# openfheorg/openfhe-development

Measured on AMD Instinct MI355X. Metric: NTT GB/s vs HBM roofline + CKKS EvalMultKeySwitch/sec, N=2^16 L=30, 1/2/4/8 GPU, higher is better.
Workload: dtype u64; 1 GPU; batched fwd+inv negacyclic NTT, N=2^16, L=30 x 60-bit limbs, 1024 polynomials per GPU (BASELINE configs[1]); global_batch=1024, parallelism=batch-sharded x1, no data-path collective

## Files before the change

### openfhe-development_amd/csrc/fhe_hip.cpp

```cpp
#include "../../include/fhe_hip.h"

#include <algorithm>
#include <cmath>
#include <cstdio>
#include <cstdlib>
#include <map>
#include <mutex>
#include <shared_mutex>
#include <string>
#include <type_traits>
#include <vector>

#include "basis_kernels.h"
#include "bfv_kernels.h"
#include "elemwise_kernels.h"
#include "host_math.h"
#include "ntt_kernels.h"
#include "ntt_static.h"
#include "ntt_row8.h"
#include "rt.h"
#include "sampler_kernels.h"
#include "blake2_kernels.h"

using namespace fhe;
// ... 447 lines not shown
    ARG_CHECK(c && graph, "fhe_graph_launch: null argument");
    RT_CHECK(rt::graph_launch((rt::graph_t)graph, (rt::stream_t)stream));
    return FHE_OK;
}
extern "C" void fhe_graph_destroy(void* graph) {
    if (graph)
        rt::graph_destroy((rt::graph_t)graph);
}

static fhe_status make_sel(const fhe_ctx* c, const uint32_t* limbIdx, uint32_t nLimbs, LimbSel* sel, const char* who) {
    if (nLimbs < 1 || nLimbs > (uint32_t)kMaxLimbs)
        return fail(FHE_ERR_ARG, std::string(who) + ": nLimbs out of range");
    for (uint32_t i = 0; i < nLimbs; ++i) {
        uint32_t l = limbIdx ? limbIdx[i] : i;
        if (l >= c->L)
            return fail(FHE_ERR_ARG, std::string(who) + ": limb index exceeds context size");
        sel->idx[i] = (uint8_t)l;
    }
    for (uint32_t i = nLimbs; i < (uint32_t)kMaxLimbs; ++i)
        sel->idx[i] = 0;
    return FHE_OK;
}
static inline uint32_t tiles_for(const fhe_ctx* c, uint64_t rows) {
    const uint64_t words = rows << c->logN;
    return (uint32_t)((words + kTile - 1) >> kTileLog);
}
#define LAUNCH_CHECK() RT_CHECK(rt::last_launch_error())

static uint32_t env_u32(const char* name, uint32_t dflt) {
    const char* v = std::getenv(name);
    return v ? (uint32_t)std::strtoul(v, nullptr, 10) : dflt;
}
constexpr bool kHandoverDefault = true;
struct NttSwitches {
    int row8 = -1, row8X1 = -1;
    uint32_t row8Batch = 0, t1 = 0;
    bool handover = kHandoverDefault;
};
static const NttSwitches& ntt_switches() {
    static const NttSwitches sw = [] {
        NttSwitches s;
        auto flag = [](const char* name) {
            const char* v = std::getenv(name);
            return v && (v[0] == '0' || v[0] == '1') ? v[0] - '0' : -1;
        };
        s.row8   = flag("FHE_NTT_ROW8");
        s.row8X1 = flag("FHE_NTT_ROW8_X1");
        if (const char* v = std::getenv("FHE_NTT_ROW8_BATCH"))
            s.row8Batch = (v[0] == '1' || v[0] == '2' || v[0] == '4') && !v[1] ? (uint32_t)(v[0] - '0') : 0u;
        if (const char* v = std::getenv("FHE_NTT_HANDOVER")) {
            s.handover = v[0] == '1' && !v[1];
            if (!s.handover && !(v[0] == '0' && !v[1]))
                fprintf(stderr, "fhe_hip: FHE_NTT_HANDOVER=%s is neither 0 nor 1: hand-over is off\n", v);
        }
        s.t1 = env_u32("FHE_NTT_T1", 0);
        return s;
    }();
    return sw;
}
static bool row8_for(uint32_t T) { return ntt_switches().row8 >= 0 ? ntt_switches().row8 == 1 : T <= 11u; }
constexpr uint32_t kRow8BatchDefault = 2;
constexpr bool kRow8X1RegionsP2 = false, kRow8X1RegionsP4 = false;
static uint32_t row8_batch_for(uint32_t T) {
    if (T != 12u)
        return 1u;
    return ntt_switches().row8Batch ? ntt_switches().row8Batch : ntt_switches().row8 >= 0 ? 1u : kRow8BatchDefault;
}
static bool row8_x1_regions(uint32_t P) {
    return ntt_switches().row8X1 >= 0 ? ntt_switches().row8X1 == 1 : (P == 2 ? kRow8X1RegionsP2 : kRow8X1RegionsP4);
}
static uint32_t ntt_t1(uint32_t logN) {
    const uint32_t forced = ntt_switches().t1;
    if (forced >= 4 && forced <= 5 && logN > (uint32_t)kTileLog && logN - forced >= 9 && logN - forced <= 12)
        return forced;
    return std::max(4u, logN - (uint32_t)kTileLog);
}

struct NttPass {
    enum Kind { Single, Column, Row };
    bool inverse = false;
    Kind kind    = Single;
    uint32_t T   = 0;
    int mode = 1;
    NttPass() = default;
    NttPass(bool inv, Kind k, uint32_t stages) : inverse(inv), kind(k), T(stages), mode(k == Row ? (inv ? 0 : 9) : 1) {}
    bool layoutA() const { return kind == Column; }
};
struct NttPasses {
// ... 122 lines not shown
    FHE_INSTANCE(FHE_PASS_IS(LA, INV, TT, MODE), FHE_LAUNCH_BARRIER((ntt_static_kernel<LA, INV, TT, MODE>), pass_tiles(*a), stream, *a))
    FHE_CASE(true, false, 4, 1) FHE_CASE(true, true, 4, 1) FHE_CASE(true, false, 5, 1) FHE_CASE(true, true, 5, 1)
    FHE_CASE(false, false, 12, 9) FHE_CASE(false, true, 12, 0) FHE_CASE(false, false, 11, 9) FHE_CASE(false, true, 11, 0)
    FHE_CASE(false, false, 10, 9) FHE_CASE(false, true, 10, 0) FHE_CASE(false, false, 9, 9) FHE_CASE(false, true, 9, 0)
    FHE_CASE(false, false, 12, 1) FHE_CASE(false, true, 12, 1)
#undef FHE_CASE
    return false;
}
static bool static_epilogue_instance(const NttPass& p, const NttPassArgs* a, void* stream) {
#define FHE_CASE(TT, MODE) \
    FHE_INSTANCE(FHE_PASS_IS(false, false, TT, MODE),                                                                                \
                 FHE_LAUNCH_AS("EPI", (ntt_static_kernel<false, false, TT, MODE, true>), pass_tiles(*a), kThreads, true, stream, *a))
    FHE_CASE(12, 9) FHE_CASE(11, 9) FHE_CASE(10, 9) FHE_CASE(9, 9) FHE_CASE(12, 1)
#undef FHE_CASE
    return false;
}
static bool static_prologue_instance(const NttPass& p, const NttPassArgs* a, void* stream) {
#define FHE_CASE(TT)                                                                                                                  \
    FHE_INSTANCE(FHE_PASS_IS(true, false, TT, 1) && !(a && a->proMode >= 2u),                                                         \
                 FHE_LAUNCH_AS("PRO", (ntt_static_kernel<true, false, TT, 1, false, 1>), pass_tiles(*a), kThreads, true, stream, *a))  \
    FHE_INSTANCE(FHE_PASS_IS(true, false, TT, 1) && a && a->proMode == 2u,                                                            \
                 FHE_LAUNCH_AS("PRO2", (ntt_static_kernel<true, false, TT, 1, false, 2>), pass_tiles(*a), kThreads, true, stream, *a)) \
    FHE_INSTANCE(FHE_PASS_IS(true, false, TT, 1) && a && a->proMode == 3u,                                                            \
                 FHE_LAUNCH_AS("PRO3", (ntt_static_kernel<true, false, TT, 1, false, 3>), pass_tiles(*a), kThreads, true, stream, *a))
    FHE_CASE(4) FHE_CASE(5)
#undef FHE_CASE
    return false;
}
static bool static_handover_instance(const NttPass& p, const NttPassArgs* a, void* stream) {
    FHE_INSTANCE(FHE_PASS_IS(true, true, 4, 1), FHE_LAUNCH_AS("HAND", (ntt_static_kernel<true, true, 4, 1, false, false, true>), pass_tiles(*a),
                                                              kThreads, true, stream, *a))
    return false;
}
static NttPassArgs row8_args(const NttPassArgs& a, uint32_t P) {
    NttPassArgs r = a;
    r.batch       = a.batch / P;
    r.rows        = r.batch * a.nLimbs;
    r.xcdSwizzle  = ((a.nLimbs << (a.logN - a.T)) % 8u == 0) ? 1u : 0u;
    return r;
}
static bool row8_instance(const NttPass& p, const NttPassArgs* a, void* stream) {
#define FHE_CASE(INV, TT, MODE)                                                                                                       \
    FHE_INSTANCE(FHE_PASS_IS(false, INV, TT, MODE), FHE_LAUNCH_BARRIER_N((r8::ntt_row8_kernel<INV, TT - 9, MODE>), a->rows << (a->logN - TT), \
                                                                         64u << (TT - 9), stream, *a))
    FHE_CASE(false, 12, 9) FHE_CASE(true, 12, 0) FHE_CASE(false, 11, 9) FHE_CASE(true, 11, 0)
    FHE_CASE(false, 10, 9) FHE_CASE(true, 10, 0) FHE_CASE(false, 9, 9) FHE_CASE(true, 9, 0)
#undef FHE_CASE
    return false;
}
static bool row8_batched_instance(const NttPass& p, uint32_t P, bool hand, const NttPassArgs* a, void* stream) {
    const bool x1p = row8_x1_regions(P);
#define FHE_CASE(INV, MODE, PP, X1P)                                                                                                  \
    FHE_INSTANCE(FHE_PASS_IS(false, INV, 12, MODE) && P == PP && x1p == X1P && !hand,                                                 \
                 FHE_LAUNCH_BARRIER_N((r8::ntt_row8_batched_kernel<INV, 3, MODE, PP, X1P>), a->rows << (a->logN - 12), 512u, stream, *a))      \
    FHE_INSTANCE(INV && FHE_PASS_IS(false, INV, 12, MODE) && P == PP && x1p == X1P && hand,                                           \
                 FHE_LAUNCH_AS("HAND", (r8::ntt_row8_batched_kernel<INV, 3, MODE, PP, X1P, INV>), a->rows << (a->logN - 12), 512u, true, stream, \
                               *a))
    FHE_CASE(false, 9, 2, false) FHE_CASE(true, 0, 2, false) FHE_CASE(false, 9, 2, true) FHE_CASE(true, 0, 2, true)
    FHE_CASE(false, 9, 4, false) FHE_CASE(true, 0, 4, false) FHE_CASE(false, 9, 4, true) FHE_CASE(true, 0, 4, true)
#undef FHE_CASE
    return false;
}
static bool poly_mul_instance(const NttPass& p, bool second, const PolyMulArgs* a, void* stream) {
#define FHE_CASE(TT)                                                                                                                \
    FHE_INSTANCE(FHE_PASS_IS(false, false, TT, 9) && !second, FHE_LAUNCH_BARRIER((poly_mul_row_a_kernel<TT>), pass_tiles(a->fwd), stream, *a)) \
    FHE_INSTANCE(FHE_PASS_IS(false, false, TT, 9) && second, FHE_LAUNCH_BARRIER((poly_mul_row_b_kernel<TT>), pass_tiles(a->fwd), stream, *a))
    FHE_CASE(12) FHE_CASE(11) FHE_CASE(10) FHE_CASE(9)
#undef FHE_CASE
    return false;
}
#undef FHE_INSTANCE
#undef FHE_PASS_IS

static bool ntt_epilogue_supported(const fhe_ctx* c) {
    const NttPasses f = ntt_passes(c, false);
    return static_epilogue_instance(f.p[f.n - 1], nullptr, nullptr);
}
static bool ntt_prologue_supported(const fhe_ctx* c) {
    const NttPasses f = ntt_passes(c, false);
    return f.n == 2 && static_prologue_instance(f.p[0], nullptr, nullptr);
}

static void fill_pass_args(const fhe_ctx* c, const NttPass& p, const uint64_t* xin, uint64_t* xout, const LimbSel& sel, uint32_t nLimbs,
                           uint32_t batch, const NttOpts& o, NttPassArgs& a) {
    a.outStride = o.dst.stride;
    a.outFirst  = o.dst.first;
    a.inStride  = o.src.stride;
    a.inFirst   = o.src.first;
    a.inDelta   = o.srcDelta;
    a.xin       = xin;
    a.x         = xout;
    a.tw        = p.inverse ? c->d_twInv : c->d_tw;
    a.twRow     = p.inverse ? c->d_twRowInv : c->d_twRow;
    a.q         = c->d_q;
    a.red       = c->d_red;
    a.fin       = c->d_fin;
    a.logN      = c->logN;
    a.T         = p.T;
    a.nLimbs    = nLimbs;
    a.rows      = batch * nLimbs;
    a.batch     = batch;
    a.nSteps = a.canonLevels = 0;
    a.canonStep              = o.canonOut ? 0u : 0xffffffffu;
    for (NttStep& st : a.steps)
        st = NttStep{0, 0, -1, 0, 0, 0, 0, 0};
    a.sel = sel;
    const uint32_t tilesPerRow = c->N >= (uint32_t)kTile ? (c->N >> kTileLog) : 1u;
    a.xcdSwizzle = (c->N >= (uint32_t)kTile && ((nLimbs * tilesPerRow) % 8u == 0)) ? 1u : 0u;
    static const NttEpilogue noEpi;
    const NttEpilogue& e = o.epi && o.epi->mode ? *o.epi : noEpi;
    a.epiMode = e.mode, a.epiSplit = e.split, a.epiAStride = e.aStride, a.epiAFirst = e.aFirst;
    a.epiA = e.A, a.epiC = e.C, a.epiOut0 = e.out0, a.epiOut1 = e.out1, a.epiADelta = e.aDelta;
    a.proMode = o.proSrcLimb ? (o.proRows ? 3 : o.proC ? 2 : 1) : 0, a.proSrcLimb = o.proSrcLimb ? *o.proSrcLimb : 0;
    a.proC = o.proSrcLimb ? o.proC : nullptr;
    a.proRows = o.proSrcLimb ? o.proRows : 0;
    for (uint32_t k = 0; k < 4; ++k)
        a.proSrcLimbs[k] = k < a.proRows ? o.proSrcLimb[k] : 0;
}
static NttPassArgs split_head(NttPassArgs& a, uint32_t n) {
    NttPassArgs h = a;
    h.batch       = n;
    h.rows        = n * a.nLimbs;
    a.xin += a.inDelta ? (int64_t)n * a.inDelta : (int64_t)(((uint64_t)n * (a.inStride ? a.inStride : a.nLimbs)) << a.logN);
    a.x += ((uint64_t)n * (a.outStride ? a.outStride : a.nLimbs)) << a.logN;
    a.batch -= n;
    a.rows = a.batch * a.nLimbs;
    return h;
}
static fhe_status launch_pass(const fhe_ctx* c, const NttPass& p, const uint64_t* xin, uint64_t* xout, const LimbSel& sel, uint32_t nLimbs,
                              uint32_t batch, void* stream, const NttOpts& o = NttOpts(), uint32_t handP = 0) {
    NttPassArgs a;
    fill_pass_args(c, p, xin, xout, sel, nLimbs, batch, o, a);
    enum { Small, Static, Epilogue, Prologue, Row8 } rest = c->logN < (uint32_t)kTileLog ? Small : Static;
    uint32_t headP = 0;
    if (o.srcDelta && rest == Small)
        return fail(FHE_ERR_UNSUPPORTED, "ntt: separately allocated towers need a ring of at least 4096");
    if (o.proSrcLimb) {
        rest = Prologue;
        if (!static_prologue_instance(p, nullptr, nullptr))
            return fail(FHE_ERR_UNSUPPORTED, "ntt: no prologue kernel for this pass shape");
    }
    else if (a.epiMode) {
        rest = Epilogue;
        if (!static_epilogue_instance(p, nullptr, nullptr))
            return fail(FHE_ERR_UNSUPPORTED, "ntt: no epilogue kernel for this pass shape");
    }
    else if (rest != Small) {
        const uint32_t P = p.kind == NttPass::Row ? row8_batch_for(p.T) : 1u;
        if (handP && !(batch >= handP && (p.layoutA() ? static_handover_instance(p, nullptr, nullptr)
                                                      : P == handP && row8_batched_instance(p, P, true, nullptr, nullptr))))
            return fail(FHE_ERR_UNSUPPORTED, "ntt: no hand-over kernel for this pass shape");
        if (handP && p.layoutA())
            headP = handP;
        else if (P > 1 && batch >= P && row8_batched_instance(p, P, handP != 0, nullptr, nullptr))
            headP = P;
        if (p.kind == NttPass::Row && row8_for(p.T) && row8_instance(p, nullptr, nullptr))
            rest = Row8;
        else if (!static_instance(p, nullptr, nullptr))
            return fail(FHE_ERR_UNSUPPORTED, "ntt: no kernel instance for this pass shape");
    }
    if (headP) {
        NttPassArgs h = split_head(a, batch / headP * headP);
        if (p.layoutA())
            static_handover_instance(p, &h, stream);
        else
            h = row8_args(h, headP), row8_batched_instance(p, headP, handP != 0, &h, stream);
    }
    if (a.batch)
        switch (rest) {
            case Static: static_instance(p, &a, stream); break;
            case Epilogue: static_epilogue_instance(p, &a, stream); break;
            case Prologue: static_prologue_instance(p, &a, stream); break;
            case Row8: a = row8_args(a, 1), row8_instance(p, &a, stream); break;
            case Small: launch_small(p, o.canonOut, a, stream); break;
        }
    LAUNCH_CHECK();
    return FHE_OK;
}

static fhe_status ntt_run(fhe_ctx* c, bool inverse, const uint64_t* xin, uint64_t* xout, const uint32_t* limbIdx, uint32_t nLimbs,
                          uint32_t batch, void* stream, const NttOpts& o = NttOpts()) {
    ARG_CHECK(c && xin && xout, "fhe_ntt: null argument");
    ARG_CHECK(batch >= 1, "fhe_ntt: batch must be >= 1");
    LimbSel sel;
    if (fhe_status s = make_sel(c, limbIdx, nLimbs, &sel, "fhe_ntt"))
        return s;
    RT_CHECK(rt::set_device(c->device));
    const NttPasses ps = ntt_passes(c, inverse);
    if (ps.n == 1)
        return launch_pass(c, ps.p[0], xin, xout, sel, nLimbs, batch, stream, o);
    const uint32_t rowP  = inverse ? row8_batch_for(ps.p[0].T) : 1u;
    const uint32_t handP = (o.canonOut && !(o.epi && o.epi->mode) && !o.proSrcLimb && ntt_switches().handover && rowP >= 2 &&
                            batch >= rowP && row8_batched_instance(ps.p[0], rowP, true, nullptr, nullptr) &&
                            static_handover_instance(ps.p[1], nullptr, nullptr))
                               ? rowP
                               : 0u;
    NttOpts first = o, second;
    first.epi = nullptr, first.canonOut = false;
    second.src = second.dst = o.dst;
    second.epi = o.epi, second.canonOut = o.canonOut;
    if (fhe_status s = launch_pass(c, ps.p[0], xin, xout, sel, nLimbs, batch, stream, first, handP))
        return s;
    return launch_pass(c, ps.p[1], xout, xout, sel, nLimbs, batch, stream, second, handP);
}

extern "C" fhe_status fhe_ntt_fwd(fhe_ctx* c, uint64_t* x, const uint32_t* li, uint32_t nl, uint32_t b, void* st) {
    return ntt_run(c, false, x, x, li, nl, b, st);
}
extern "C" fhe_status fhe_ntt_inv(fhe_ctx* c, uint64_t* x, const uint32_t* li, uint32_t nl, uint32_t b, void* st) {
    return ntt_run(c, true, x, x, li, nl, b, st);
}
extern "C" fhe_status fhe_ntt_fwd_oop(fhe_ctx* c, const uint64_t* xi, uint64_t* xo, const uint32_t* li, uint32_t nl,
                                      uint32_t b, void* st) {
    return ntt_run(c, false, xi, xo, li, nl, b, st);
}
extern "C" fhe_status fhe_ntt_inv_oop(fhe_ctx* c, const uint64_t* xi, uint64_t* xo, const uint32_t* li, uint32_t nl,
                                      uint32_t b, void* st) {
    return ntt_run(c, true, xi, xo, li, nl, b, st);
}

extern "C" size_t fhe_poly_mul_workspace_bytes(const fhe_ctx* c, uint32_t nLimbs, uint32_t batch) {
    return c ? (((size_t)2 * batch * nLimbs) << c->logN) * 8 : 0;
}
extern "C" fhe_status fhe_poly_mul(fhe_ctx* c, const uint64_t* a, const uint64_t* b, uint64_t* out, const uint32_t* limbIdx,
                                   uint32_t nLimbs, uint32_t batch, void* wsv, size_t wsBytes, void* stream) {
    ARG_CHECK(c && a && b && out && wsv, "fhe_poly_mul: null argument");
    ARG_CHECK(batch >= 1, "fhe_poly_mul: batch must be >= 1");
    ARG_CHECK(wsBytes >= fhe_poly_mul_workspace_bytes(c, nLimbs, batch), "fhe_poly_mul: workspace too small");
    LimbSel sel;
    if (fhe_status s = make_sel(c, limbIdx, nLimbs, &sel, "fhe_poly_mul"))
        return s;
    RT_CHECK(rt::set_device(c->device));
    uint64_t* wa = (uint64_t*)wsv;
    uint64_t* wb = wa + (((size_t)batch * nLimbs) << c->logN);
    const NttPasses f = ntt_passes(c, false), i = ntt_passes(c, true);
    if (f.n != 2 || !poly_mul_instance(f.p[1], false, nullptr, nullptr)) {
// ... 3936 lines not shown
```

### openfhe-development_amd/csrc/ntt_kernels.h

```cpp
#ifndef FHE_NTT_KERNELS_H
#define FHE_NTT_KERNELS_H
#include "modarith.h"
#include "launch.h"

namespace fhe {

constexpr int kTileLog  = 12;
constexpr int kTile     = 1 << kTileLog;
constexpr int kThreads  = 256;
constexpr int kMaxLimbs = 256;

struct alignas(16) TwPair {
    uint64_t w, wp;
};

struct LimbSel {
    uint8_t idx[kMaxLimbs];
};

struct NttStep {
    int8_t fI;
    int8_t Fj;
    int8_t bHi;
    int8_t bLo;
// ... 4 lines not shown
};

struct NttPassArgs {
    const uint64_t* xin;
    uint64_t* x;
    const TwPair* tw;
    const TwPair* twRow;
    const uint64_t* q;
    const uint64_t* red;
    const TwPair* fin;
    uint32_t logN;
    uint32_t T;
    uint32_t nLimbs;
    uint32_t rows;
    uint32_t batch;
    uint32_t nSteps;
    uint32_t canonLevels;
    uint32_t canonStep;
    uint32_t xcdSwizzle;
    uint32_t inStride;
    uint32_t inFirst;
    uint32_t outStride;
    uint32_t outFirst;
    NttStep steps[6];
    LimbSel sel;
    uint32_t epiMode, epiSplit, epiAStride, epiAFirst;
    const uint64_t* epiA;
    const TwPair* epiC;
    uint64_t *epiOut0, *epiOut1;
    uint32_t proMode, proSrcLimb;
    const TwPair* proC;
    uint32_t proRows, proSrcLimbs[4];
    int64_t inDelta, epiADelta;
};
FHE_HD uint64_t switch_modulus_word(uint64_t v, uint64_t qs, uint64_t halfQs, uint64_t qn) {
    if (qn > qs)
        return v + ((v > halfQs) ? (qn - qs) : 0);
    uint64_t bv = (v > halfQs) ? (qs - qn) : 0;
    uint64_t av = v;
    if (av >= qn)
        av %= qn;
    if (bv >= qn)
        bv %= qn;
    return (av < bv) ? av + qn - bv : av - bv;
}

FHE_HD uint32_t lds_sigma(uint32_t I) {
    return I ^ ((I >> 4) & 31u);
}

FHE_HD void bfly_fwd(uint64_t& a, uint64_t& b, const TwPair w, uint64_t nq, uint64_t twoq) {
    uint64_t X = csub(a, twoq);
    uint64_t T = mul_shoup_lazy_nq(b, w.w, w.wp, nq);
    a          = X + T;
    b          = X - T + twoq;
}
FHE_HD void bfly_inv(uint64_t& a, uint64_t& b, const TwPair w, uint64_t nq, uint64_t twoq) {
    uint64_t u = a, v = b;
    a          = csub(u + v, twoq);
    b          = mul_shoup_lazy_nq(u - v + twoq, w.w, w.wp, nq);
}
FHE_HD void bfly_inv_last(uint64_t& a, uint64_t& b, const TwPair nInv, const TwPair w1nInv, uint64_t nq,
                          uint64_t twoq) {
    uint64_t u = a, v = b;
    a          = mul_shoup_lazy_nq(u + v, nInv.w, nInv.wp, nq);
    b          = mul_shoup_lazy_nq(u - v + twoq, w1nInv.w, w1nInv.wp, nq);
// ... 216 lines not shown
```

### openfhe-development_amd/csrc/ntt_row8.h

```cpp
#ifndef FHE_NTT_ROW8_H
#define FHE_NTT_ROW8_H
#include "ntt_static.h"
#include "ntt_bfly8_pinned.h"
#include <type_traits>
#if defined(__HIP_DEVICE_COMPILE__) && !defined(FHE_NO_BFLY_ASM)
namespace fhe {
namespace r8 {
#define FHE_BK 1
namespace bk1 {
#include "ntt_bfly8_banked.h"
}
#undef FHE_BK
#define FHE_BK 2
namespace bk2 {
#include "ntt_bfly8_banked.h"
}
#undef FHE_BK
#define FHE_BK 3
namespace bk3 {
#include "ntt_bfly8_banked.h"
}
#undef FHE_BK
}
}
// ... 214 lines not shown
}
template <bool UNI, int NB, bool SWEEP>
FHE_HD void fwd_step(uint64_t (&r)[8], const TwPair* tw, uint32_t hi, uint32_t F, uint32_t logN, const BflyConst c, uint32_t inBound) {
    uint32_t bnd[8];
    for (int k = 0; k < 8; ++k)
        bnd[k] = inBound;
    TwPair w2[4], w1[4], w0[4];
    if constexpr (NB >= 1) load_tw<UNI, 2>(w2, tw, hi, F, logN);
    if constexpr (NB >= 2) load_tw<UNI, 1>(w1, tw, hi, F, logN);
    if constexpr (SWEEP && NB >= 1)
        red4_a<2>(r, c, bnd);
    if constexpr (NB >= 1) fwd_stage<UNI, 2>(r, w2, c, bnd);
    if constexpr (NB >= 3) load_tw<UNI, 0>(w0, tw, hi, F, logN);
    if constexpr (NB >= 2) fwd_stage<UNI, 1>(r, w1, c, bnd);
    if constexpr (NB >= 3) fwd_stage<UNI, 0>(r, w0, c, bnd);
}
template <bool UNI, int NB, bool LAZY>
FHE_HD void inv_step(uint64_t (&r)[8], const TwPair* tw, uint32_t hi, uint32_t F, uint32_t logN, const BflyConst c) {
    uint32_t bnd[8];
    for (int k = 0; k < 8; ++k)
        bnd[k] = 3;
    TwPair w2[4], w1[4], w0[4];
    if constexpr (NB >= 3) load_tw<UNI, 0>(w0, tw, hi, F, logN);
    if constexpr (NB >= 2) load_tw<UNI, 1>(w1, tw, hi, F, logN);
    if constexpr (NB >= 1 && NB < 3) load_tw<UNI, 2>(w2, tw, hi, F, logN);
    if constexpr (NB >= 3) inv_stage<UNI, NB, 0>(r, w0, c, bnd);
    if constexpr (NB >= 3) load_tw<UNI, 2>(w2, tw, hi, F, logN);
    if constexpr (NB >= 2) inv_stage<UNI, NB, 1>(r, w1, c, bnd);
    if constexpr (NB >= 1) inv_stage<UNI, NB, 2>(r, w2, c, bnd);
    if constexpr (!LAZY && NB >= 1)
        inv_end<NB>(r, c, bnd);
}

template <int WB, int BIN>
struct FwdSched {
    static constexpr int TA = WB;
    static constexpr int stages(int i) { return i == 0 ? TA : 3; }
    static constexpr int before(int i) {
        int b = BIN;
        for (int j = 0; j < i; ++j)
            b = (b + 3 * stages(j) <= 16) ? b + 3 * stages(j) : 2 + 3 * stages(j);
        return b;
    }
    static constexpr bool sweep(int i) { return before(i) + 3 * stages(i) > 16; }
    static constexpr int out = before(4);
};

struct TileAt {
    uint32_t tb, rit, tr;
};
FHE_DEV TileAt tile_at(const NttPassArgs& a, uint32_t vt, uint32_t trLog, bool swz) {
    uint32_t tile = vt;
    if (swz) {
        const uint32_t xcd = vt & 7u, i = vt >> 3;
        const uint32_t b = i % a.batch, pairIdx = i / a.batch;
        const uint32_t pair = pairIdx * 8u + xcd;
        tile = ((b * a.nLimbs + (pair >> trLog)) << trLog) + (pair & ((1u << trLog) - 1u));
    }
    const uint32_t row = tile >> trLog;
    return TileAt{row / a.nLimbs, row % a.nLimbs, tile & ((1u << trLog) - 1u)};
}

#if defined(__HIP_DEVICE_COMPILE__)
#define FHE_R8_OPAQUE_V(x) asm volatile("" : "+v"(x))
#else
#define FHE_R8_OPAQUE_V(x) ((void)0)
#endif
#define FHE_R8_LANE()                 \
    uint32_t tq_ = t;                 \
// ... 218 lines not shown
    if constexpr (NB >= 3) load_tw<UNI, 0>(w0, tw, hi, F, logN);
    FHE_R8_BANKS(p)
        if constexpr (NB >= 2) fwd_stage<UNI, 1, p>(r[p], w1, c, bnd[p]);
    FHE_R8_BANKS_END
    FHE_R8_BANKS(p)
        if constexpr (NB >= 3) fwd_stage<UNI, 0, p>(r[p], w0, c, bnd[p]);
    FHE_R8_BANKS_END
}
template <bool UNI, int NB, bool LAZY, int P, bool HAND = false>
FHE_HD void inv_step_b(uint64_t (&r)[P][8], const TwPair* tw, uint32_t hi, uint32_t F, uint32_t logN, const BflyConst c) {
    uint32_t bnd[P][8];
    for (int p = 0; p < P; ++p)
        for (int k = 0; k < 8; ++k)
            bnd[p][k] = 3;
    TwPair w2[4], w1[4], w0[4];
    if constexpr (NB >= 3) load_tw<UNI, 0>(w0, tw, hi, F, logN);
    if constexpr (NB >= 2) load_tw<UNI, 1>(w1, tw, hi, F, logN);
    if constexpr (NB >= 1 && NB < 3) load_tw<UNI, 2>(w2, tw, hi, F, logN);
    FHE_R8_BANKS(p)
        if constexpr (NB >= 3) inv_stage<UNI, NB, 0, p>(r[p], w0, c, bnd[p]);
    FHE_R8_BANKS_END
    static_assert(!HAND || (NB == 3 && LAZY), "row8 hand-over: the boundary stage is the last of the full step that closes a lazy-out pass");
    if constexpr (NB >= 3 && !HAND) load_tw<UNI, 2>(w2, tw, hi, F, logN);
    FHE_R8_BANKS(p)
        if constexpr (NB >= 2) inv_stage<UNI, NB, 1, p>(r[p], w1, c, bnd[p]);
    FHE_R8_BANKS_END
    FHE_R8_BANKS(p)
        if constexpr (HAND) inv_stage_hand<p>(r[p], c, bnd[p]);
        else if constexpr (NB >= 1) inv_stage<UNI, NB, 2, p>(r[p], w2, c, bnd[p]);
        if constexpr (!LAZY && NB >= 1) inv_end<NB, p>(r[p], c, bnd[p]);
    FHE_R8_BANKS_END
}

template <bool INV, int WB, int MODE, int P, bool X1P, bool HAND = false>
FHE_DEV void ntt_row8_batched_core(const NttPassArgs& a, uint64_t* lds) {
    static_assert(WB == 3, "row8 batched: 8 waves per tile (12 stages): the banked blocks exist for full radix-8 steps only");
    static_assert(P >= 2 && P <= 4, "row8 batched: register banks 0..3");
    static_assert(!(INV && MODE != 0), "row8: the inverse pass that ends a transform is ntt_static.h's");
    static_assert(!HAND || INV, "row8 hand-over: the inverse pass only");
    constexpr uint32_t tileLog = 9u + (uint32_t)WB;
    constexpr uint32_t threads = 64u << WB;
    constexpr int WLOW         = 3 - WB;
    constexpr uint32_t x1Set   = X1P ? (uint32_t)kRegion << WB : 0u;
    const uint32_t t     = FHE_TID;
    const uint32_t wv    = FHE_UNIFORM(t >> 6);
    const uint32_t logN  = a.logN;
    const uint32_t trLog = logN - tileLog;
    uint64_t* reg = lds + (size_t)wv * kRegion;
    uint64_t r[P][8];
    const TileAt at      = tile_at(a, FHE_BID, trLog, a.xcdSwizzle != 0);
    const uint32_t jbase = at.tr << tileLog;
    const uint32_t rit   = at.rit;
    const uint32_t tb0   = at.tb * (uint32_t)P;
    const uint64_t inRow  = a.inStride ? ((uint64_t)tb0 * a.inStride + a.inFirst + rit) : ((uint64_t)tb0 * a.nLimbs + rit);
    const uint64_t outRow = a.outStride ? ((uint64_t)tb0 * a.outStride + a.outFirst + rit) : ((uint64_t)tb0 * a.nLimbs + rit);
    const uint32_t limb = FHE_UNIFORM(a.sel.idx[rit]);
    const uint64_t q    = FHE_ULOAD64(a.q, limb);
    const uint64_t twoq = q << 1, nq = 0 - q;
    const TwPair* tw    = a.tw + ((uint64_t)limb << logN);
    const uint64_t redc = FHE_ULOAD64(a.red, limb);
    const BflyConst c{(uint32_t)nq, (uint32_t)(nq >> 32), q, twoq, 0 - twoq, twoq + q, (uint32_t)redc, (uint32_t)(redc >> 32)};
    const uint64_t* src = (a.inDelta ? a.xin + (int64_t)tb0 * a.inDelta + ((uint64_t)(a.inFirst + rit) << logN) : a.xin + (inRow << logN)) + jbase;
    uint64_t* dst       = a.x + (outRow << logN) + jbase;
    const int64_t inStep  = a.inDelta ? a.inDelta : (int64_t)((uint64_t)(a.inStride ? a.inStride : a.nLimbs) << logN);
    const int64_t outStep = (int64_t)((uint64_t)(a.outStride ? a.outStride : a.nLimbs) << logN);
    auto x1 = [](int rr) { return (uint32_t)kRegion * ((uint32_t)rr >> WLOW) + (64u << WB) * ((uint32_t)rr & ((1u << WLOW) - 1u)); };
#define FHE_R8_LANE()                 \
    uint32_t tq_ = t;                 \
    FHE_R8_OPAQUE_V(tq_);             \
    const uint32_t l = tq_ & 63u, lhi = l >> 3, llo = l & 7u; \
    (void)lhi, (void)llo
#define FHE_R8_XCHG(pp, WBASE, WR, RBASE, RD)             \
    do {                                                  \
        FHE_WAVE_SYNC();                                  \
        uint64_t* Lw_ = (WBASE);                          \
        _Pragma("unroll") for (int k = 0; k < 8; ++k)     \
            FHE_LDS_ST(Lw_[WR], r[pp][k]);                \
        FHE_WAVE_SYNC();                                  \
        const uint64_t* Lr_ = (RBASE);                    \
        _Pragma("unroll") for (int k = 0; k < 8; ++k)     \
            FHE_LDS_LD(r[pp][k], Lr_[RD]);                \
    } while (0)

    if constexpr (!INV) {
        using S = FwdSched<WB, (MODE == 9 ? 2 : MODE)>;
        {
            FHE_R8_LANE();
            FHE_R8_BANKS(p)
                const uint64_t* s0 = src + (int64_t)p * inStep + tq_;
#pragma unroll
                for (int k = 0; k < 8; ++k)
                    r[p][k] = FHE_GLD(&s0[threads * (uint32_t)k]);
            FHE_R8_BANKS_END
        }
        fwd_step_b<true, WB, S::sweep(0), P>(r, tw, at.tr, 6 + WB, logN, c, S::sweep(0) ? 2u : (uint32_t)S::before(0));
        {
            FHE_R8_LANE();
            FHE_R8_BANKS(p)
                if constexpr (!X1P && p > 0)
                    FHE_SSYNC();
                uint64_t* Lw = lds + (uint32_t)p * x1Set + tq_;
#pragma unroll
                for (int k = 0; k < 8; ++k)
                    FHE_LDS_ST(Lw[x1(k)], r[p][k]);
                FHE_SSYNC();
                const uint64_t* Lr = reg + (uint32_t)p * x1Set + l;
#pragma unroll
                for (int k = 0; k < 8; ++k)
                    FHE_LDS_LD(r[p][k], Lr[64 * k]);
            FHE_R8_BANKS_END
        }
        fwd_step_b<true, 3, S::sweep(1), P>(r, tw, (jbase >> 9) + wv, 6, logN, c, S::sweep(1) ? 2u : (uint32_t)S::before(1));
        {
            FHE_R8_LANE();
            FHE_R8_BANKS(p)
                FHE_R8_XCHG(p, reg + l, 72 * k, reg + 72u * lhi + llo, 8 * k);
            FHE_R8_BANKS_END
            fwd_step_b<false, 3, S::sweep(2), P>(r, tw, (jbase >> 6) + (wv << 3) + lhi, 3, logN, c, S::sweep(2) ? 2u : (uint32_t)S::before(2));
        }
        {
            FHE_R8_LANE();
            FHE_R8_BANKS(p)
                FHE_R8_XCHG(p, reg + fc3(lhi) + llo, 33 * k, reg + fc3(lhi) + 33u * llo, k);
            FHE_R8_BANKS_END
            fwd_step_b<false, 3, S::sweep(3), P>(r, tw, (jbase >> 3) + (wv << 6) + l, 0, logN, c, S::sweep(3) ? 2u : (uint32_t)S::before(3));
        }
        {
            FHE_R8_LANE();
// ... 40 lines not shown
        inv_step_b<true, 3, false, P>(r, tw, (jbase >> 9) + wv, 6, logN, c);
        {
            FHE_R8_LANE();
            FHE_R8_BANKS(p)
                if constexpr (!X1P && p > 0)
                    FHE_SSYNC();
                FHE_WAVE_SYNC();
                uint64_t* Lw = reg + (uint32_t)p * x1Set + l;
#pragma unroll
                for (int k = 0; k < 8; ++k)
                    FHE_LDS_ST(Lw[64 * k], r[p][k]);
                FHE_SSYNC();
                const uint64_t* Lr = lds + (uint32_t)p * x1Set + tq_;
#pragma unroll
                for (int k = 0; k < 8; ++k)
                    FHE_LDS_LD(r[p][k], Lr[x1(k)]);
            FHE_R8_BANKS_END
            inv_step_b<true, WB, true, P, HAND>(r, tw, at.tr, 6 + WB, logN, c);
            FHE_R8_BANKS(p)
                uint64_t* d0 = dst + (int64_t)p * outStep + tq_;
#pragma unroll
                for (int k = 0; k < 8; ++k)
                    FHE_GST(&d0[threads * (uint32_t)k], r[p][k]);
            FHE_R8_BANKS_END
        }
    }
#undef FHE_R8_XCHG
#undef FHE_R8_LANE
}
#undef FHE_R8_BANKS
#undef FHE_R8_BANKS_END

constexpr int batched_waves(int P, bool X1P) { return X1P ? (P == 2 ? 4 : 2) : (P == 2 ? 6 : 4); }
template <bool INV, int WB, int MODE, int P, bool X1P, bool HAND = false>
FHE_GLOBAL void FHE_LAUNCH_BOUNDS2(64 << WB, batched_waves(P, X1P)) ntt_row8_batched_kernel(const NttPassArgs a) {
    FHE_SHARED_U64(lds, (X1P ? P : 1) * (1 << WB) * kRegion);
    ntt_row8_batched_core<INV, WB, MODE, P, X1P, HAND>(a, lds);
}

}
}
#endif
```

### openfhe-development_amd/csrc/ntt_static.h

```cpp
#ifndef FHE_NTT_STATIC_H
#define FHE_NTT_STATIC_H
#include "ntt_kernels.h"
#include "ntt_inv_plan16.h"

#if defined(__HIP_DEVICE_COMPILE__) && !defined(FHE_NO_BFLY_ASM)
#include "ntt_bfly_pinned.h"
#define FHE_PINNED_ASM 1
#endif

namespace fhe {

#ifndef FHE_PINNED_ASM
struct BflyConst {
    uint32_t nql, nqh;
    uint64_t q, twoq, ntwoq, threeq;
    uint32_t redM, redR;
};
struct BflyZero {
    uint32_t z0, z1;
};
#endif
constexpr int kFwdGrow = 3;

FHE_HD uint64_t shoup_trunc(uint64_t y, const TwPair w, uint64_t nq) {
// ... 700 lines not shown
        else if constexpr (I == P::nst - 1 && !P::stageLast) {                                                    \
            store_result(r, jrel, ks);                                                                            \
        }                                                                                                         \
        else {                                                                                                    \
            if constexpr (I > 0 || P::stageFirst || RAWIN)                                                        \
                FHE_SSYNC();                                       \
            uint64_t* L = lds + lds_pad(Ib);                                                 \
            _Pragma("unroll") for (int k = 0; k < 16; ++k) FHE_LDS_ST(L[lds_pad((uint32_t)k << fI)], r[k]);                  \
            FHE_SSYNC();                                                                                           \
        }                                                                                                         \
    }
    FHE_STATIC_STEP(0)
    FHE_STATIC_STEP(1)
    FHE_STATIC_STEP(2)
#undef FHE_STATIC_STEP
#undef FHE_SHARED_TW_TO_LDS

    if constexpr (P::stageLast && !RAWOUT) {
        lane_geom_s<LA, T, 8>(t, S, Ib, jrel, ks);
        const uint64_t* L = lds + lds_pad(Ib);
#pragma unroll
        for (int k = 0; k < 16; ++k)
            FHE_LDS_LD(r[k], L[lds_pad((uint32_t)k << 8)]);
        store_result(r, jrel, ks);
    }
}

template <bool LA, bool INV, int T, int MODE, bool EPI = false, int PRO = 0, bool HAND = false>
FHE_DEV void ntt_static_body(const NttPassArgs& a, uint32_t bid, uint64_t* lds) {
    uint64_t r[16];
    ntt_static_core<LA, INV, T, MODE, EPI, false, false, PRO, HAND>(a, bid, lds, r);
}

template <bool LA, bool INV, int T, int MODE, bool EPI = false, int PRO = 0, bool HAND = false>
FHE_GLOBAL void FHE_LAUNCH_BOUNDS(kThreads) ntt_static_kernel(const NttPassArgs a) {
    using P = SPlan<LA, INV, T>;
    constexpr bool needsLds = P::nst > 1 || P::stageFirst || P::stageLast;
#ifndef FHE_ABL_LDSPAD
#define FHE_ABL_LDSPAD 0
#endif
    FHE_SHARED_U64(lds, needsLds ? kLdsPadWords + kSharedTwWords + FHE_ABL_LDSPAD : 1);
    ntt_static_body<LA, INV, T, MODE, EPI, PRO, HAND>(a, FHE_BID, lds);
}


struct PolyMulArgs {
    NttPassArgs fwd;
    NttPassArgs inv;
    uint64_t* aEval;
    const LimbConst* lc;
};
template <int T>
FHE_GLOBAL void FHE_LAUNCH_BOUNDS(kThreads) poly_mul_row_a_kernel(const PolyMulArgs g) {
    FHE_SHARED_U64(lds, kLdsPadWords + kSharedTwWords);
    uint64_t r[16];
    ntt_static_core<false, false, T, 9, false, false, true>(g.fwd, FHE_BID, lds, r);
    uint64_t* dst = g.aEval + ((uint64_t)FHE_BID << kTileLog) + FHE_TID;
#pragma unroll
    for (int k = 0; k < 16; ++k)
        dst[(uint32_t)k * kThreads] = r[k];
}
template <int T>
FHE_GLOBAL void FHE_LAUNCH_BOUNDS2(kThreads, 4) poly_mul_row_b_kernel(const PolyMulArgs g) {
    FHE_SHARED_U64(lds, kLdsPadWords + kSharedTwWords);
    uint64_t r[16];
    ntt_static_core<false, false, T, 9, false, false, true>(g.fwd, FHE_BID, lds, r);
    {
        const uint32_t tilesPerRow = 1u << (g.fwd.logN - (uint32_t)kTileLog);
        const uint32_t row         = FHE_BID / tilesPerRow;
        const LimbConst lc         = g.lc[FHE_UNIFORM(g.fwd.sel.idx[row % g.fwd.nLimbs])];
        const uint64_t* av         = g.aEval + ((uint64_t)FHE_BID << kTileLog) + FHE_TID;
#pragma unroll
        for (int g4 = 0; g4 < 4; ++g4) {
            uint64_t x[4];
// ... 17 lines not shown
```

Before: 2321 GB/s.

## Split forward N=2^16 NTT as 6 column stages plus 10 row stages

```diff
diff --git a/openfhe-development_amd/csrc/fhe_hip.cpp b/openfhe-development_amd/csrc/fhe_hip.cpp
--- a/openfhe-development_amd/csrc/fhe_hip.cpp
+++ b/openfhe-development_amd/csrc/fhe_hip.cpp
@@ -503,10 +503,12 @@
     return v ? (uint32_t)std::strtoul(v, nullptr, 10) : dflt;
 }
 constexpr bool kHandoverDefault = true;
+constexpr bool kSplit6Default = true;
 struct NttSwitches {
     int row8 = -1, row8X1 = -1;
     uint32_t row8Batch = 0, t1 = 0;
     bool handover = kHandoverDefault;
+    bool split6 = kSplit6Default;
 };
 static const NttSwitches& ntt_switches() {
     static const NttSwitches sw = [] {
@@ -525,6 +527,12 @@
                 fprintf(stderr, "fhe_hip: FHE_NTT_HANDOVER=%s is neither 0 nor 1: hand-over is off\n", v);
         }
         s.t1 = env_u32("FHE_NTT_T1", 0);
+        if (const char* v = std::getenv("FHE_NTT_SPLIT6")) {
+            const std::string w = v;
+            s.split6 = w == "1" || w == "fwd";
+            if (!s.split6 && w != "0" && w != "inv")
+                fprintf(stderr, "fhe_hip: FHE_NTT_SPLIT6=%s is none of 0, 1, fwd, inv: the 6 + 10 split is off\n", v);
+        }
         return s;
     }();
     return sw;
@@ -713,6 +721,11 @@
                                                               kThreads, true, stream, *a))
     return false;
 }
+static bool static_split6_instance(const NttPass& p, const NttPassArgs* a, void* stream) {
+    FHE_INSTANCE(FHE_PASS_IS(true, false, 4, 1), FHE_LAUNCH_AS("SPLIT6", (ntt_static_kernel<true, false, 4, 1, false, 0, false, true>),
+                                                               pass_tiles(*a), kThreads, true, stream, *a))
+    return false;
+}
 static NttPassArgs row8_args(const NttPassArgs& a, uint32_t P) {
     NttPassArgs r = a;
     r.batch       = a.batch / P;
@@ -729,8 +742,14 @@
 #undef FHE_CASE
     return false;
 }
-static bool row8_batched_instance(const NttPass& p, uint32_t P, bool hand, const NttPassArgs* a, void* stream) {
+static bool row8_batched_instance(const NttPass& p, uint32_t P, bool hand, bool split6, const NttPassArgs* a, void* stream) {
     const bool x1p = row8_x1_regions(P);
+    if (split6) {
+        FHE_INSTANCE(FHE_PASS_IS(false, false, 12, 9) && P == 2 && !x1p && !hand,
+                     FHE_LAUNCH_AS("SPLIT6", (r8::ntt_row8_batched_kernel<false, 3, 9, 2, false, false, true>), a->rows << (a->logN - 12), 512u,
+                                   true, stream, *a))
+        return false;
+    }
 #define FHE_CASE(INV, MODE, PP, X1P)                                                                                                  \
     FHE_INSTANCE(FHE_PASS_IS(false, INV, 12, MODE) && P == PP && x1p == X1P && !hand,                                                 \
                  FHE_LAUNCH_BARRIER_N((r8::ntt_row8_batched_kernel<INV, 3, MODE, PP, X1P>), a->rows << (a->logN - 12), 512u, stream, *a))      \
@@ -795,6 +814,7 @@
     a.proMode = o.proSrcLimb ? (o.proRows ? 3 : o.proC ? 2 : 1) : 0, a.proSrcLimb = o.proSrcLimb ? *o.proSrcLimb : 0;
     a.proC = o.proSrcLimb ? o.proC : nullptr;
     a.proRows = o.proSrcLimb ? o.proRows : 0;
+    a.split6Batch = 0;
     for (uint32_t k = 0; k < 4; ++k)
         a.proSrcLimbs[k] = k < a.proRows ? o.proSrcLimb[k] : 0;
 }
@@ -809,7 +829,7 @@
     return h;
 }
 static fhe_status launch_pass(const fhe_ctx* c, const NttPass& p, const uint64_t* xin, uint64_t* xout, const LimbSel& sel, uint32_t nLimbs,
-                              uint32_t batch, void* stream, const NttOpts& o = NttOpts(), uint32_t handP = 0) {
+                              uint32_t batch, void* stream, const NttOpts& o = NttOpts(), uint32_t handP = 0, uint32_t splitP = 0) {
     NttPassArgs a;
     fill_pass_args(c, p, xin, xout, sel, nLimbs, batch, o, a);
     enum { Small, Static, Epilogue, Prologue, Row8 } rest = c->logN < (uint32_t)kTileLog ? Small : Static;
@@ -829,11 +849,20 @@
     else if (rest != Small) {
         const uint32_t P = p.kind == NttPass::Row ? row8_batch_for(p.T) : 1u;
         if (handP && !(batch >= handP && (p.layoutA() ? static_handover_instance(p, nullptr, nullptr)
-                                                      : P == handP && row8_batched_instance(p, P, true, nullptr, nullptr))))
+                                                      : P == handP && row8_batched_instance(p, P, true, false, nullptr, nullptr))))
             return fail(FHE_ERR_UNSUPPORTED, "ntt: no hand-over kernel for this pass shape");
+        if (splitP && !(batch >= splitP && (p.layoutA() ? static_split6_instance(p, nullptr, nullptr)
+                                                        : P == splitP && row8_batched_instance(p, P, false, true, nullptr, nullptr))))
+            return fail(FHE_ERR_UNSUPPORTED, "ntt: no kernel of the 6 + 10 split for this pass shape");
+        if (splitP && p.layoutA()) {
+            a.split6Batch = batch / splitP * splitP;
+            static_split6_instance(p, &a, stream);
+            LAUNCH_CHECK();
+            return FHE_OK;
+        }
         if (handP && p.layoutA())
             headP = handP;
-        else if (P > 1 && batch >= P && row8_batched_instance(p, P, handP != 0, nullptr, nullptr))
+        else if (P > 1 && batch >= P && row8_batched_instance(p, P, handP != 0, splitP != 0, nullptr, nullptr))
             headP = P;
         if (p.kind == NttPass::Row && row8_for(p.T) && row8_instance(p, nullptr, nullptr))
             rest = Row8;
@@ -845,7 +874,7 @@
         if (p.layoutA())
             static_handover_instance(p, &h, stream);
         else
-            h = row8_args(h, headP), row8_batched_instance(p, headP, handP != 0, &h, stream);
+            h = row8_args(h, headP), row8_batched_instance(p, headP, handP != 0, splitP != 0, &h, stream);
     }
     if (a.batch)
         switch (rest) {
@@ -872,17 +901,24 @@
         return launch_pass(c, ps.p[0], xin, xout, sel, nLimbs, batch, stream, o);
     const uint32_t rowP  = inverse ? row8_batch_for(ps.p[0].T) : 1u;
     const uint32_t handP = (o.canonOut && !(o.epi && o.epi->mode) && !o.proSrcLimb && ntt_switches().handover && rowP >= 2 &&
-                            batch >= rowP && row8_batched_instance(ps.p[0], rowP, true, nullptr, nullptr) &&
+                            batch >= rowP && row8_batched_instance(ps.p[0], rowP, true, false, nullptr, nullptr) &&
                             static_handover_instance(ps.p[1], nullptr, nullptr))
                                ? rowP
                                : 0u;
+    const NttSwitches& sw = ntt_switches();
+    const uint32_t fwdP   = inverse ? 1u : row8_batch_for(ps.p[1].T);
+    const uint32_t splitP = (!inverse && sw.split6 && c->logN == 16u && !(o.epi && o.epi->mode) && !o.proSrcLimb && sw.row8 < 0 && !sw.t1 &&
+                             fwdP == 2u && batch >= fwdP && static_split6_instance(ps.p[0], nullptr, nullptr) &&
+                             row8_batched_instance(ps.p[1], fwdP, false, true, nullptr, nullptr))
+                                ? fwdP
+                                : 0u;
     NttOpts first = o, second;
     first.epi = nullptr, first.canonOut = false;
     second.src = second.dst = o.dst;
     second.epi = o.epi, second.canonOut = o.canonOut;
-    if (fhe_status s = launch_pass(c, ps.p[0], xin, xout, sel, nLimbs, batch, stream, first, handP))
-        return s;
-    return launch_pass(c, ps.p[1], xout, xout, sel, nLimbs, batch, stream, second, handP);
+    if (fhe_status s = launch_pass(c, ps.p[0], xin, xout, sel, nLimbs, batch, stream, first, handP, splitP))
+        return s;
+    return launch_pass(c, ps.p[1], xout, xout, sel, nLimbs, batch, stream, second, handP, splitP);
 }
 
 extern "C" fhe_status fhe_ntt_fwd(fhe_ctx* c, uint64_t* x, const uint32_t* li, uint32_t nl, uint32_t b, void* st) {
diff --git a/openfhe-development_amd/csrc/ntt_kernels.h b/openfhe-development_amd/csrc/ntt_kernels.h
--- a/openfhe-development_amd/csrc/ntt_kernels.h
+++ b/openfhe-development_amd/csrc/ntt_kernels.h
@@ -60,6 +60,7 @@
     const TwPair* proC;
     uint32_t proRows, proSrcLimbs[4];
     int64_t inDelta, epiADelta;
+    uint32_t split6Batch;
 };
 FHE_HD uint64_t switch_modulus_word(uint64_t v, uint64_t qs, uint64_t halfQs, uint64_t qn) {
     if (qn > qs)
diff --git a/openfhe-development_amd/csrc/ntt_row8.h b/openfhe-development_amd/csrc/ntt_row8.h
--- a/openfhe-development_amd/csrc/ntt_row8.h
+++ b/openfhe-development_amd/csrc/ntt_row8.h
@@ -270,9 +270,9 @@
         inv_end<NB>(r, c, bnd);
 }
 
-template <int WB, int BIN>
+template <int WB, int BIN, int TA_ = WB>
 struct FwdSched {
-    static constexpr int TA = WB;
+    static constexpr int TA = TA_;
     static constexpr int stages(int i) { return i == 0 ? TA : 3; }
     static constexpr int before(int i) {
         int b = BIN;
@@ -557,8 +557,22 @@
     FHE_R8_BANKS_END
 }
 
-template <bool INV, int WB, int MODE, int P, bool X1P, bool HAND = false>
+template <int P>
+FHE_HD void fwd_step_last_b(uint64_t (&r)[P][8], const TwPair* tw, uint32_t hi, uint32_t F, uint32_t logN, const BflyConst c, uint32_t inBound) {
+    uint32_t bnd[P][8];
+    for (int p = 0; p < P; ++p)
+        for (int k = 0; k < 8; ++k)
+            bnd[p][k] = inBound;
+    TwPair w0[4];
+    load_tw<true, 0>(w0, tw, hi, F, logN);
+    FHE_R8_BANKS(p)
+        fwd_stage<true, 0, p>(r[p], w0, c, bnd[p]);
+    FHE_R8_BANKS_END
+}
+
+template <bool INV, int WB, int MODE, int P, bool X1P, bool HAND = false, bool SPLIT = false>
 FHE_DEV void ntt_row8_batched_core(const NttPassArgs& a, uint64_t* lds) {
+    static_assert(!SPLIT || (!INV && P == 2), "row8 6 + 10 split: the forward pass at two polynomials per workgroup only");
     static_assert(WB == 3, "row8 batched: 8 waves per tile (12 stages): the banked blocks exist for full radix-8 steps only");
     static_assert(P >= 2 && P <= 4, "row8 batched: register banks 0..3");
     static_assert(!(INV && MODE != 0), "row8: the inverse pass that ends a transform is ntt_static.h's");
@@ -608,7 +622,7 @@
     } while (0)
 
     if constexpr (!INV) {
-        using S = FwdSched<WB, (MODE == 9 ? 2 : MODE)>;
+        using S = FwdSched<WB, (MODE == 9 ? 2 : MODE), (SPLIT ? 1 : WB)>;
         {
             FHE_R8_LANE();
             FHE_R8_BANKS(p)
@@ -618,7 +632,12 @@
                     r[p][k] = FHE_GLD(&s0[threads * (uint32_t)k]);
             FHE_R8_BANKS_END
         }
-        fwd_step_b<true, WB, S::sweep(0), P>(r, tw, at.tr, 6 + WB, logN, c, S::sweep(0) ? 2u : (uint32_t)S::before(0));
+        if constexpr (SPLIT) {
+            static_assert(!S::sweep(0), "row8 6 + 10 split: the one stage of the w-step takes what the column pass leaves (below 2q)");
+            fwd_step_last_b<P>(r, tw, at.tr, 6 + WB, logN, c, (uint32_t)S::before(0));
+        }
+        else
+            fwd_step_b<true, WB, S::sweep(0), P>(r, tw, at.tr, 6 + WB, logN, c, S::sweep(0) ? 2u : (uint32_t)S::before(0));
         {
             FHE_R8_LANE();
             FHE_R8_BANKS(p)
@@ -725,12 +744,12 @@
 #undef FHE_R8_BANKS_END
 
 constexpr int batched_waves(int P, bool X1P) { return X1P ? (P == 2 ? 4 : 2) : (P == 2 ? 6 : 4); }
-template <bool INV, int WB, int MODE, int P, bool X1P, bool HAND = false>
+template <bool INV, int WB, int MODE, int P, bool X1P, bool HAND = false, bool SPLIT = false>
 FHE_GLOBAL void FHE_LAUNCH_BOUNDS2(64 << WB, batched_waves(P, X1P)) ntt_row8_batched_kernel(const NttPassArgs a) {
     FHE_SHARED_U64(lds, (X1P ? P : 1) * (1 << WB) * kRegion);
-    ntt_row8_batched_core<INV, WB, MODE, P, X1P, HAND>(a, lds);
-}
-
-}
-}
-#endif
+    ntt_row8_batched_core<INV, WB, MODE, P, X1P, HAND, SPLIT>(a, lds);
+}
+
+}
+}
+#endif
diff --git a/openfhe-development_amd/csrc/ntt_static.h b/openfhe-development_amd/csrc/ntt_static.h
--- a/openfhe-development_amd/csrc/ntt_static.h
+++ b/openfhe-development_amd/csrc/ntt_static.h
@@ -756,14 +756,110 @@
     ntt_static_core<LA, INV, T, MODE, EPI, false, false, PRO, HAND>(a, bid, lds, r);
 }
 
-template <bool LA, bool INV, int T, int MODE, bool EPI = false, int PRO = 0, bool HAND = false>
+FHE_DEV uint32_t static_tile(const NttPassArgs& a, uint32_t bid, uint32_t tilesPerRow) {
+    uint32_t tile = bid;
+    if (a.xcdSwizzle) {
+        const uint32_t xcd = tile & 7u, i = tile >> 3;
+        const uint32_t b = i % a.batch, pairIdx = i / a.batch;
+        const uint32_t pair = pairIdx * 8u + xcd;
+        tile = (b * a.nLimbs + pair / tilesPerRow) * tilesPerRow + pair % tilesPerRow;
+    }
+    return tile;
+}
+FHE_DEV void ntt_col6_fwd_body(const NttPassArgs& a, uint32_t tile, uint64_t* lds) {
+    const uint32_t t    = FHE_TID;
+    const uint32_t logN = a.logN;
+    const uint32_t tilesPerRow = 1u << (logN - (uint32_t)kTileLog);
+    const uint32_t row = tile / tilesPerRow, tr = tile % tilesPerRow;
+    const uint32_t jbase = tr << 6;
+    const uint64_t S     = (uint64_t)1 << (logN - 6u);
+    const uint32_t tb = row / a.nLimbs, rit = row % a.nLimbs;
+    const uint64_t inRow  = a.inStride ? ((uint64_t)tb * a.inStride + a.inFirst + rit) : (uint64_t)row;
+    const uint64_t outRow = a.outStride ? ((uint64_t)tb * a.outStride + a.outFirst + rit) : (uint64_t)row;
+    const uint32_t limb = FHE_UNIFORM(a.sel.idx[rit]);
+    const uint64_t q    = FHE_ULOAD64(a.q, limb);
+    const uint64_t twoq = q << 1, nq = 0 - q;
+    TwSrc ts;
+    ts.tw         = a.tw + ((uint64_t)limb << logN);
+    ts.fin        = nullptr;
+    ts.rowLane    = nullptr;
+    ts.shared     = nullptr;
+    ts.sharedLane = 0;
+    const uint64_t redc = FHE_ULOAD64(a.red, limb);
+    const BflyConst c{(uint32_t)nq, (uint32_t)(nq >> 32), q, twoq, 0 - twoq, twoq + q, (uint32_t)redc, (uint32_t)(redc >> 32)};
+    BflyZero z{0, 0};
+#ifdef FHE_PINNED_ASM
+    asm volatile("v_mov_b32 %0, 0\n\tv_mov_b32 %1, 0" : "={v65}"(z.z0), "={v81}"(z.z1));
+#endif
+    const uint64_t* src = (a.inDelta ? a.xin + (int64_t)tb * a.inDelta + ((uint64_t)(a.inFirst + rit) << logN) : a.xin + (inRow << logN)) + jbase;
+    uint64_t* dst       = a.x + (outRow << logN) + jbase;
+    const uint32_t wv = FHE_UNIFORM(t >> 6), l = t & 63u;
+    uint64_t r[16];
+    {
+        const uint64_t* s0 = src + (uint64_t)wv * S + l;
+#pragma unroll
+        for (int k = 0; k < 16; ++k)
+            r[k] = FHE_GLD(&s0[(uint64_t)(4 * k) * S]);
+    }
+    using P4 = SPlan<true, false, 4>;
+    static_assert(!P4::sweep(0, 1) && P4::outBound(1) == 13, "the first four stages take a canonical input to 13q without a sweep");
+    run_step<true, false, 4, 0, false, false>(r, ts, jbase, logN, c, z, 1u);
+    {
+        uint64_t* Lw = lds + wv * 64u + l;
+#pragma unroll
+        for (int k = 0; k < 16; ++k)
+            FHE_LDS_ST(Lw[256 * k], r[k]);
+        FHE_SSYNC();
+        const uint64_t* Lr = lds + wv * 1024u + l;
+#pragma unroll
+        for (int k = 0; k < 16; ++k)
+            FHE_LDS_LD(r[k], Lr[64 * k]);
+    }
+    uint32_t bnd[16];
+    for (int k = 0; k < 16; ++k)
+        bnd[k] = (k & 2) ? (uint32_t)P4::outBound(1) : 2u;
+    TwPair w1[8], w0[8];
+    {
+        const uint64_t* p1 = reinterpret_cast<const uint64_t*>(ts.tw + 16u + 4u * wv);
+        const uint64_t* p0 = reinterpret_cast<const uint64_t*>(ts.tw + 32u + 8u * wv);
+#if defined(__HIP_DEVICE_COMPILE__)
+        asm volatile("" : "+s"(p1), "+s"(p0));
+#endif
+#pragma unroll
+        for (int g = 0; g < 4; ++g)
+            w1[g] = TwPair{FHE_ULOAD64(p1, 2 * g), FHE_ULOAD64(p1, 2 * g + 1)};
+#pragma unroll
+        for (int g = 0; g < 8; ++g)
+            w0[g] = TwPair{FHE_ULOAD64(p0, 2 * g), FHE_ULOAD64(p0, 2 * g + 1)};
+    }
+    run_red8_a<1>(r, c);
+    run_stage<false, true, 1, 0>(r, w1, c, z, bnd);
+    run_stage<false, true, 0, 0>(r, w0, c, z, bnd);
+    run_red16(r, c);
+    uint64_t* d0 = dst + (uint64_t)(16u * wv) * S + l;
+#pragma unroll
+    for (int k = 0; k < 16; ++k)
+        FHE_GST(&d0[(uint64_t)k * S], r[k]);
+}
+
+template <bool LA, bool INV, int T, int MODE, bool EPI = false, int PRO = 0, bool HAND = false, bool SPLIT = false>
 FHE_GLOBAL void FHE_LAUNCH_BOUNDS(kThreads) ntt_static_kernel(const NttPassArgs a) {
     using P = SPlan<LA, INV, T>;
     constexpr bool needsLds = P::nst > 1 || P::stageFirst || P::stageLast;
+    static_assert(!SPLIT || (LA && !INV && T == 4 && MODE == 1 && !EPI && !PRO && !HAND && !needsLds),
+                  "the 6 + 10 split exists for the plain forward 4-stage column pass only");
 #ifndef FHE_ABL_LDSPAD
 #define FHE_ABL_LDSPAD 0
 #endif
-    FHE_SHARED_U64(lds, needsLds ? kLdsPadWords + kSharedTwWords + FHE_ABL_LDSPAD : 1);
+    FHE_SHARED_U64(lds, SPLIT ? kTile : needsLds ? kLdsPadWords + kSharedTwWords + FHE_ABL_LDSPAD : 1);
+    if constexpr (SPLIT) {
+        const uint32_t tilesPerRow = 1u << (a.logN - (uint32_t)kTileLog);
+        const uint32_t tile        = static_tile(a, FHE_BID, tilesPerRow);
+        if (tile / tilesPerRow / a.nLimbs < a.split6Batch) {
+            ntt_col6_fwd_body(a, tile, lds);
+            return;
+        }
+    }
     ntt_static_body<LA, INV, T, MODE, EPI, PRO, HAND>(a, FHE_BID, lds);
 }
 
```

New measurement: 2350 GB/s (median of 6 runs). 1.01x the previous value.
